# lzhangbj/DualVar

Hardware: AMD Instinct MI355X
Metric: clips/sec (whole node), S3D-G 8x112^2 SimCLR pretrain step (higher is better)
Workload: dtype fp32

## Files before the change

dualvar_amd/csrc/batchnorm.hip:

```cpp
#include "streaming.hpp"

namespace {

struct BnFinalize {
  const float* gamma; const float* beta; float eps, momentum;
  float* running_mean; float* running_var; float* mean; float* invstd; float* scale; float* shift;
};
template <typename F>
__device__ __forceinline__ void bn_finalize_channel(const F& f, int c, float mean, float M2, float cnt) {
  const float var = M2 / cnt;
  const float invstd = rsqrtf(var + f.eps);
  f.mean[c] = mean;
  f.invstd[c] = invstd;
  const float sc = f.gamma[c] * invstd;
  f.scale[c] = sc;
  f.shift[c] = f.beta[c] - mean * sc;
  if (f.running_mean) {
    f.running_mean[c] = (1.f - f.momentum) * f.running_mean[c] + f.momentum * mean;
    const float unbiased = cnt > 1.f ? M2 / (cnt - 1.f) : var;
    f.running_var[c] = (1.f - f.momentum) * f.running_var[c] + f.momentum * unbiased;
  }
}
__device__ __forceinline__ void bn_combine_ranks(const float* stats, int R, int stride, int C, int c, float& mean, float& M2, float& cnt) {
  float n = 0.f, S = 0.f;
  for (int r = 0; r < R; ++r) { n += stats[r * stride + 2 * C]; S += stats[r * stride + c]; }
  const float mu = S / n;
  float q = 0.f;
  for (int r = 0; r < R; ++r) {
    float n_r = stats[r * stride + 2 * C];
    float d = stats[r * stride + c] / n_r - mu;
    q += stats[r * stride + C + c] + n_r * d * d;
  }
// ... 101 lines not shown
      if (res) o += r[e];
      if (flags & DV_RELU) o = fmaxf(o, 0.f);
      v[e] = (c0 + e < C) ? o : 0.f;
    }
    Pack16<T>::store(y + (size_t)row * ldy + c0, v);
  }
}

template <typename T>
__global__ void bn_apply_kernel(const T* __restrict__ x, int ldx, const float* __restrict__ scale,
                                const float* __restrict__ shift, const T* __restrict__ res, int ldr,
                                T* __restrict__ y, int ldy, uint32_t total, int C, FastDiv fcv, int flags) {
  bn_apply_body<T>(x, ldx, scale, shift, res, ldr, y, ldy, total, C, fcv, flags, blockIdx.x, gridDim.x);
}

template <typename T>
__global__ void bn_apply_multi_kernel(const dv_bn_item* __restrict__ items, int n) {
  uint32_t bid = blockIdx.x, nblk;
  const int i = find_item(n, bid, nblk, [&](int k) { return items[k].blk_apply; });
  const dv_bn_item& it = items[i];
  constexpr int V = DT<T>::VEC;
  const int CP = (it.C + 7) & ~7;
  bn_apply_body<T>((const T*)it.x, it.ldx, it.scale, it.shift, (const T*)it.residual, it.ldr, (T*)it.y, it.ldy,
                   (uint32_t)(it.M * (CP / V)), it.C, make_fastdiv((uint32_t)(CP / V)), it.fwd_flags, bid, nblk);
}

struct GateOnLoad {
  const float* g; const float* dm; FastDiv fS; int ldg; float invS;
};

template <typename T>
struct PlainDy {
  static constexpr int V = DT<T>::VEC, kRows = 0;
  static constexpr bool kPooled = false;
  struct Pend {};
  const T* dy; int lddy;
  __device__ __forceinline__ void load(int64_t r, int c0, float (&g)[V], Pend&) const { Pack16<T>::load(dy + r * lddy + c0, g); }
  __device__ __forceinline__ void finish(int64_t, int, float (&)[V], Pend&) const {}
};

template <typename T, bool ROW_FIRST>
struct GatedDy {
  static constexpr int V = DT<T>::VEC, kRows = V == 4 ? 2 : 1;
  static constexpr bool kPooled = false;
  struct Pend { float gv[V], dv[V]; };
  const T* dy; int lddy; GateOnLoad ga;
  __device__ __forceinline__ void gate_row(int64_t r, int c0, Pend& p) const {
    const size_t go = (size_t)fd_div((uint32_t)r, ga.fS) * ga.ldg;
    load_params<V>(ga.g + go, c0, p.gv);
    load_params<V>(ga.dm + go, c0, p.dv);
  }
  __device__ __forceinline__ void load(int64_t r, int c0, float (&g)[V], Pend& p) const {
    if (ROW_FIRST && ga.g) gate_row(r, c0, p);
    Pack16<T>::load(dy + r * lddy + c0, g);
  }
  __device__ __forceinline__ void finish(int64_t r, int c0, float (&g)[V], Pend& p) const {
    if (!ga.g) return;
    if (!ROW_FIRST) gate_row(r, c0, p);
#pragma unroll
    for (int e = 0; e < V; ++e) g[e] = as_stored<T>(gate_grad(g[e], p.gv[e], p.dv[e], ga.invS));
  }
};

template <typename T>
__global__ __launch_bounds__(kThreads) void bn_bwd_reduce_kernel(const T* __restrict__ dy, int lddy, const T* __restrict__ y, int ldy,
                                     const T* __restrict__ x, int ldx, const float* __restrict__ mean,
                                     const float* __restrict__ invstd, int64_t M, int C, int CP, int flags,
                                     int64_t rows_per_block, float* __restrict__ sums_all, int n_rep, float* __restrict__ ws) {
  bn_bwd_reduce_body<T>(PlainDy<T>{dy, lddy}, y, ldy, x, ldx, mean, invstd, M, C, CP, flags, rows_per_block, sums_all, n_rep,
                        blockIdx.x, nullptr, nullptr, ws, gridDim.x);
}

template <typename T>
__global__ __launch_bounds__(kThreads) void bn_bwd_reduce_multi_kernel(const dv_bn_item* __restrict__ items, int n) {
  uint32_t bid = blockIdx.x, nblk;
  const int i = find_item(n, bid, nblk, [&](int k) { return items[k].blk_red; });
  const dv_bn_item& it = items[i];
  const int CP = (it.C + 7) & ~7;
  const int64_t rpb = (it.M + nblk - 1) / nblk;
  bn_bwd_reduce_body<T>(PlainDy<T>{(const T*)it.dy, it.lddy}, (const T*)it.y, it.ldy, (const T*)it.x, it.ldx, it.mean,
                        it.invstd, it.M, it.C, CP, it.bwd_flags, rpb, it.sums, it.n_rep, bid, it.scale, it.shift, it.red_ws, nblk);
}

__device__ __forceinline__ GateOnLoad gate_of_item(const int32_t* __restrict__ gate_off, int i, const float* g, const float* dm,
                                                   const FastDiv& fS, int ldg) {
  const int off = gate_off[i];
  GateOnLoad ga;
  ga.g = off >= 0 ? g + off : nullptr;
  ga.dm = off >= 0 ? dm + off : nullptr;
  ga.fS = fS; ga.ldg = ldg; ga.invS = 1.f / (float)fS.d;
  return ga;
}

template <typename T>
__global__ __launch_bounds__(kThreads) void bn_bwd_reduce_multi_gated_kernel(const dv_bn_item* __restrict__ items, int n,
                                                                            const int32_t* __restrict__ gate_off,
                                                                            const float* __restrict__ g, const float* __restrict__ dm,
                                                                            FastDiv fS, int ldg) {
  uint32_t bid = blockIdx.x, nblk;
  const int i = find_item(n, bid, nblk, [&](int k) { return items[k].blk_red; });
  const dv_bn_item& it = items[i];
  const int CP = (it.C + 7) & ~7;
  const int64_t rpb = (it.M + nblk - 1) / nblk;
  bn_bwd_reduce_body<T>(GatedDy<T, true>{(const T*)it.dy, it.lddy, gate_of_item(gate_off, i, g, dm, fS, ldg)}, (const T*)it.y, it.ldy,
                        (const T*)it.x, it.ldx, it.mean, it.invstd, it.M, it.C, CP, it.bwd_flags, rpb, it.sums, it.n_rep, bid,
                        it.scale, it.shift, it.red_ws, nblk);
}

template <typename T>
__global__ void bn_bwd_apply_kernel(const T* __restrict__ dy, int lddy, const T* __restrict__ y, int ldy,
                                    const T* __restrict__ x, int ldx, const float* __restrict__ mean,
                                    const float* __restrict__ invstd, const float* __restrict__ gamma,
                                    const float* __restrict__ sums_g, int rep_g, float inv_count, float dscale,
                                    float* dgamma, float* dbeta, T* __restrict__ dx, int lddx,
                                    T* __restrict__ dres, int lddres, uint32_t total, int C, int CP, FastDiv fcv,
                                    int flags) {
  bn_bwd_apply_body<T>(PlainDy<T>{dy, lddy}, y, ldy, x, ldx, mean, invstd, gamma, sums_g, rep_g, inv_count, dscale, dgamma,
                       dbeta, dx, lddx, dres, lddres, total, C, CP, fcv, flags, blockIdx.x, gridDim.x, nullptr, nullptr);
}

template <typename T>
__global__ void bn_bwd_apply_multi_kernel(const dv_bn_item* __restrict__ items, int n) {
  uint32_t bid = blockIdx.x, nblk;
  const int i = find_item(n, bid, nblk, [&](int k) { return items[k].blk_bapply; });
  const dv_bn_item& it = items[i];
  constexpr int V = DT<T>::VEC;
  const int CP = (it.C + 7) & ~7;
  bn_bwd_apply_body<T>(PlainDy<T>{(const T*)it.dy, it.lddy}, (const T*)it.y, it.ldy, (const T*)it.x, it.ldx, it.mean, it.invstd,
                       it.gamma, it.sums, it.n_rep, it.inv_count, it.dparam_scale, it.dgamma, it.dbeta, (T*)it.dx, it.lddx,
                       (T*)it.dres, it.lddres, (uint32_t)(it.M * (CP / V)), it.C, CP, make_fastdiv((uint32_t)(CP / V)),
                       it.bwd_flags, bid, nblk, it.scale, it.shift);
}

template <typename T>
__global__ void bn_bwd_apply_multi_gated_kernel(const dv_bn_item* __restrict__ items, int n, const int32_t* __restrict__ gate_off,
                                                const float* __restrict__ g, const float* __restrict__ dm, FastDiv fS, int ldg) {
  uint32_t bid = blockIdx.x, nblk;
  const int i = find_item(n, bid, nblk, [&](int k) { return items[k].blk_bapply; });
  const dv_bn_item& it = items[i];
  constexpr int V = DT<T>::VEC;
  const int CP = (it.C + 7) & ~7;
  bn_bwd_apply_body<T>(GatedDy<T, false>{(const T*)it.dy, it.lddy, gate_of_item(gate_off, i, g, dm, fS, ldg)}, (const T*)it.y, it.ldy,
                       (const T*)it.x, it.ldx, it.mean, it.invstd, it.gamma, it.sums, it.n_rep, it.inv_count, it.dparam_scale,
                       it.dgamma, it.dbeta, (T*)it.dx, it.lddx, (T*)it.dres, it.lddres, (uint32_t)(it.M * (CP / V)), it.C, CP,
                       make_fastdiv((uint32_t)(CP / V)), it.bwd_flags, bid, nblk, it.scale, it.shift);
}

}

__global__ void bn_eval_coeffs_kernel(const float* __restrict__ gamma, const float* __restrict__ beta,
                                      const float* __restrict__ rm, const float* __restrict__ rv, float eps, int C, int CP,
                                      float* __restrict__ scale, float* __restrict__ shift) {
  const int c = blockIdx.x * blockDim.x + threadIdx.x;
  if (c >= CP) return;
  float sc = 0.f, sh = 0.f;
  if (c < C) {
    sc = gamma[c] * rsqrtf(rv[c] + eps);
    sh = beta[c] - rm[c] * sc;
  }
  scale[c] = sc;
  shift[c] = sh;
}

extern "C" int dv_bn_eval_coeffs(const float* gamma, const float* beta, const float* running_mean, const float* running_var,
                                 float eps, int32_t C, float* scale, float* shift, void* stream) {
  if (!gamma || !beta || !running_mean || !running_var || !scale || !shift || C <= 0) return DV_EINVAL;
  const int CP = cp8(C);
  hipLaunchKernelGGL(bn_eval_coeffs_kernel, dim3((CP + 127) / 128), dim3(128), 0, ST(stream), gamma, beta, running_mean,
                     running_var, eps, C, CP, scale, shift);
  return dv_launch_status();
}

__global__ void bn_rows_partials_kernel(const float* __restrict__ x, int ldx, int M, int C, float* __restrict__ part) {
  const int c = blockIdx.x * blockDim.x + threadIdx.x;
  if (c >= C) return;
// ... 189 lines not shown
```

dualvar_amd/csrc/conv.hip:

```cpp
#include "conv_common.hpp"
#include "../../include/dualvar_conv_pair.h"

static int w3_rows(int n) { return (n + 127) / 128 * 128; }
static int64_t w3_bytes(int n, int ktot) { return (int64_t)((ktot + 15) / 16) * 2 * w3_rows(n) * 48; }

namespace {
__global__ __launch_bounds__(256) void pack_w3_kernel(const float* __restrict__ base, unsigned char* __restrict__ out_base,
                                                      const dv_w3_desc* __restrict__ descs, const int2* __restrict__ block_map) {
  const int2 bm = block_map[blockIdx.x];
  const dv_w3_desc d = descs[bm.x];
  const int npad = (d.N + 127) / 128 * 128;
  const long long unit = (long long)bm.y + threadIdx.x;
  const long long units = (long long)((d.Ktot + 15) / 16) * 2 * npad;
  if (unit >= units) return;
  const int n = (int)(unit % npad);
  const int kh = (int)(unit / npad), k0 = (kh >> 1) * 16 + (kh & 1) * 8;
  float v[8];
#pragma unroll
  for (int e = 0; e < 8; ++e) v[e] = (n < d.N && k0 + e < d.Ktot) ? base[d.src_off + (long long)n * d.Ktot + k0 + e] : 0.f;
  const Split3 s3 = split3(v);
  bf16x8* o = reinterpret_cast<bf16x8*>(out_base + d.dst_off + unit * 48);
  o[0] = s3.hi; o[1] = s3.mid; o[2] = s3.lo;
}
}

extern "C" int64_t dv_w3_bytes(int32_t rows, int32_t ktot) { return rows > 0 && ktot > 0 ? w3_bytes(rows, ktot) : 0; }

extern "C" int dv_pack_w3(const float* base, void* out_base, const dv_w3_desc* descs, const int32_t* block_map, int32_t n_blocks,
                          void* stream) {
  if (!base || !out_base || !descs || !block_map || n_blocks <= 0) return DV_EINVAL;
  hipLaunchKernelGGL(pack_w3_kernel, dim3(n_blocks), dim3(256), 0, (hipStream_t)stream, base, (unsigned char*)out_base, descs,
                     reinterpret_cast<const int2*>(block_map));
  return dv_launch_status();
}

static int pick_bn(int np) {
  if (np <= 32) return 32;
  if (np <= 64) return 64;
  int w128 = (np + 127) / 128 * 128, w64 = (np + 63) / 64 * 64;
  return (w128 <= w64) ? 128 : 64;
}

static int pick_bm(int M, int ntn) {
  return ((int64_t)((M + 127) / 128) * ntn >= 1024) ? 128 : 64;
}

static void pick_tile(int dtype, int M, int NP, int& bm, int& bn) {
  bn = pick_bn(NP);
  const int ntn = (NP + bn - 1) / bn;
  bm = pick_bm(M, ntn);
  if (dtype == DV_F32 && !f32_exact() && bm == 128 && bn == 64 && (int64_t)((M + 255) / 256) * ntn >= 512) bm = 256;
  constexpr int fill = 256;
  if (bm == 64) {
// ... 559 lines not shown
```

dualvar_amd/csrc/elementwise.hip:

```cpp
#include "streaming.hpp"

namespace {

template <typename T>
__global__ void ingest_kernel(const float* __restrict__ x, T* __restrict__ y, int N, int C, int T_, int H, int W,
                              int64_t sxn, int ldy, const float* mean3, const float* istd3,
                              const int* perm, int n_seg, int pad, int Hp, int Wp) {
  const int64_t total = (int64_t)N * T_ * H * W;
  const int64_t plane = (int64_t)H * W;
  const int seg = n_seg > 0 ? T_ / n_seg : T_;
  for (int64_t i = blockIdx.x * (int64_t)blockDim.x + threadIdx.x; i < total; i += (int64_t)gridDim.x * blockDim.x) {
    int64_t hw = i % plane;
    int64_t nt = i / plane;
    int t = (int)(nt % T_);
    int n = (int)(nt / T_);
    int ts = t;
    if (perm) ts = perm[n * n_seg + t / seg] * seg + t % seg;
    const float* src = x + (int64_t)n * sxn + (int64_t)ts * plane + hw;
    float v[4] = {0.f, 0.f, 0.f, 0.f};
    for (int c = 0; c < C && c < 4; ++c) {
      float a = src[(int64_t)c * T_ * plane];
      if (mean3) a = (a - mean3[c]) * istd3[c];
      v[c] = a;
    }
// ... 42 lines not shown
  if (row >= R) return;
  const int lane = threadIdx.x & 63;
  float s = 0.f;
  for (int d = lane; d < D; d += 64) { float v = x[(size_t)row * D + d]; s += v * v; }
  s = wave_sum(s);
  const float nrm = fmaxf(sqrtf(s), eps);
  for (int d = lane; d < D; d += 64) y[(size_t)row * D + d] = x[(size_t)row * D + d] / nrm;
  if (lane == 0) norm[row] = nrm;
}
__global__ void l2norm_bwd_kernel(const float* __restrict__ dy, const float* __restrict__ y,
                                  const float* __restrict__ norm, int R, int D, float* __restrict__ dx) {
  const int row = blockIdx.x * (blockDim.x >> 6) + (threadIdx.x >> 6);
  if (row >= R) return;
  const int lane = threadIdx.x & 63;
  float s = 0.f;
  for (int d = lane; d < D; d += 64) s += dy[(size_t)row * D + d] * y[(size_t)row * D + d];
  s = wave_sum(s);
  const float inv = 1.f / norm[row];
  for (int d = lane; d < D; d += 64)
    dx[(size_t)row * D + d] = (dy[(size_t)row * D + d] - y[(size_t)row * D + d] * s) * inv;
}
__global__ void relu_bwd_kernel(const float* __restrict__ dy, const float* __restrict__ y, int64_t n, float* __restrict__ dx) {
  for (int64_t i = blockIdx.x * (int64_t)blockDim.x + threadIdx.x; i < n; i += (int64_t)gridDim.x * blockDim.x)
    dx[i] = y[i] > 0.f ? dy[i] : 0.f;
}
__global__ void mean_kernel(const float* __restrict__ x, int n, float* __restrict__ out) {
  __shared__ float sh[8];
  float s = 0.f;
  for (int i = threadIdx.x; i < n; i += blockDim.x) s += x[i];
  s = block_sum(s, sh);
  if (threadIdx.x == 0) out[0] = s / (float)n;
}

template <typename CT>
__global__ void pack_dgrad_kernel(const float* __restrict__ master, CT* __restrict__ dst,
                                  const dv_pack_desc* __restrict__ descs, const int* __restrict__ bmap) {
  const dv_pack_desc d = descs[bmap[2 * blockIdx.x]];
  const int c = bmap[2 * blockIdx.x + 1];
  const int rowlen = d.taps * d.cout_pitch;
  const float* src = master + d.src_off;
  CT* out = dst + d.dst_off + (int64_t)c * rowlen;
  for (int i = threadIdx.x; i < rowlen; i += blockDim.x) {
    const int tap = i / d.cout_pitch, n = i % d.cout_pitch;
    float v = 0.f;
    if (n < d.Cout) v = src[((int64_t)n * d.taps + tap) * d.cin_pitch + c];
    out[i] = (CT)v;
  }
}

}

extern "C" int dv_abi_version(void) { return DV_ABI_VERSION; }

extern "C" int dv_check_device(void) {
  int dev = 0;
  if (hipGetDevice(&dev) != hipSuccess) return DV_EUNSUPPORTED;
  hipDeviceProp_t prop;
  if (hipGetDeviceProperties(&prop, dev) != hipSuccess) return DV_EUNSUPPORTED;
  const char* a = prop.gcnArchName;
  return (a[0] == 'g' && a[1] == 'f' && a[2] == 'x' && a[3] == '9' && a[4] == '5' && a[5] == '0') ? DV_OK : DV_EUNSUPPORTED;
}

extern "C" int dv_ingest_ncdhw(int32_t dtype, const float* x, void* y, int32_t N, int32_t C, int32_t T_, int32_t H,
                               int32_t W, int64_t sxn, int32_t ldy, const float* mean3, const float* istd3,
                               const int32_t* perm, int32_t n_seg, void* stream) {
  if (!x || !y || N <= 0 || C <= 0 || C > 4 || ldy < 4 || ldy % 4) return DV_EINVAL;
  if (perm && (n_seg <= 0 || T_ % n_seg)) return DV_EINVAL;
  if ((mean3 == nullptr) != (istd3 == nullptr)) return DV_EINVAL;
  const int64_t total = (int64_t)N * T_ * H * W;
  DISPATCH_T(dtype, hipLaunchKernelGGL((ingest_kernel<T>), dim3(grid_for(total)), dim3(kThreads), 0, ST(stream), x,
                                       (T*)y, N, C, T_, H, W, sxn, ldy, mean3, istd3, perm, n_seg, 0, H, W));
  return dv_launch_status();
}

extern "C" int dv_ingest_ncdhw_pad(int32_t dtype, const float* x, void* y, int32_t N, int32_t C, int32_t T_, int32_t H,
                                   int32_t W, int64_t sxn, int32_t ldy, const float* mean3, const float* istd3,
                                   const int32_t* perm, int32_t n_seg, int32_t pad, void* stream) {
  if (!x || !y || N <= 0 || C <= 0 || C > 4 || ldy < 4 || ldy % 4 || pad < 0) return DV_EINVAL;
  if (perm && (n_seg <= 0 || T_ % n_seg)) return DV_EINVAL;
// ... 69 lines not shown
```

dualvar_amd/csrc/pool.hip:

```cpp
#include "streaming.hpp"

namespace {

__device__ __forceinline__ uint32_t xcd_block() { return (blockIdx.x & 7u) * (gridDim.x >> 3) + (blockIdx.x >> 3); }
static inline int grid8_for(int64_t work_items, int max_blocks) { return (grid_for(work_items, max_blocks) + 7) & ~7; }

struct PoolArgs {
  int N, Ti, Hi, Wi, C, CP;
  int To, Ho, Wo;
  int kt, kh, kw, st, sh, sw, pt, ph, pw;
  int ldx, ldy;
  FastDiv fcv, fWo, fHo, fTo, fWi, fHi, fTi;
};

template <typename T>
__global__ void maxpool_fwd_kernel(PoolArgs a, const T* __restrict__ x, T* __restrict__ y, uint8_t* __restrict__ idx) {
  constexpr int V = DT<T>::VEC;
  const uint32_t CV = a.fcv.d;
  const uint32_t total = (uint32_t)a.N * a.To * a.Ho * a.Wo * CV;
  for (uint32_t i = xcd_block() * blockDim.x + threadIdx.x; i < total; i += gridDim.x * blockDim.x) {
    uint32_t m, cvi, q, wo_, ho_, to_, n_;
    fd_divmod(i, a.fcv, m, cvi);
    const int c0 = (int)cvi * V;
    fd_divmod(m, a.fWo, q, wo_);
// ... 187 lines not shown
                                            uint32_t m_in, int c0, float (&g)[DT<T>::VEC]) {
  constexpr int V = DT<T>::VEC;
  uint32_t q, wi_, hi_, ti_, n_;
  fd_divmod(m_in, a.fWi, q, wi_);
  fd_divmod(q, a.fHi, q, hi_);
  fd_divmod(q, a.fTi, n_, ti_);
  const int n = (int)n_;
  const int st1 = a.st - 1, sh1 = a.sh - 1, sw1 = a.sw - 1;
  const int tn = (int)ti_ + a.pt, hn = (int)hi_ + a.ph, wn = (int)wi_ + a.pw;
  const int t_hi = min(tn >> st1, a.To - 1), t_lo = max((tn - a.kt + 1 + st1) >> st1, 0);
  const int h_hi = min(hn >> sh1, a.Ho - 1), h_lo = max((hn - a.kh + 1 + sh1) >> sh1, 0);
  const int w_hi = min(wn >> sw1, a.Wo - 1), w_lo = max((wn - a.kw + 1 + sw1) >> sw1, 0);
  for (int to = t_hi; to >= t_lo; --to) {
    const int dt = tn - to * a.st;
    for (int ho = h_hi; ho >= h_lo; --ho) {
      const int dh = hn - ho * a.sh;
      for (int wo = w_hi; wo >= w_lo; --wo) {
        const uint32_t tap = (uint32_t)((dt * a.kh + dh) * a.kw + wn - wo * a.sw);
        const int64_t mo = (int64_t)((n * a.To + to) * a.Ho + ho) * a.Wo + wo;
        float d[V];
        Pack16<T>::load(dyp + mo * a.ldy + c0, d);
        const uint8_t* ip = idx + mo * a.CP + c0;
#pragma unroll
        for (int e = 0; e < V; ++e)
          if (ip[e] == tap) g[e] += d[e];
      }
    }
  }
}

template <typename T>
struct PooledDy {
  static constexpr int V = DT<T>::VEC, kRows = 0;
  static constexpr bool kPooled = true;
  struct Pend {};
  const PoolArgs& a; const T* dyp; const uint8_t* idx;
  __device__ __forceinline__ void load(int64_t r, int c0, float (&g)[V], Pend&) const {
#pragma unroll
    for (int e = 0; e < V; ++e) g[e] = 0.f;
    pool_gather<T>(a, dyp, idx, (uint32_t)r, c0, g);
  }
  __device__ __forceinline__ void finish(int64_t, int, float (&)[V], Pend&) const {}
};

template <typename T>
__global__ __launch_bounds__(kThreads) void bn_bwd_reduce_maxpool_kernel(PoolArgs a, const T* __restrict__ dyp, const uint8_t* __restrict__ idx,
                                             const T* __restrict__ x, const float* __restrict__ mean,
                                             const float* __restrict__ invstd, const float* __restrict__ scale,
                                             const float* __restrict__ shift, int64_t M, int C, int CP, int64_t rows_per_block,
                                             float* __restrict__ sums_all, int n_rep) {
  bn_bwd_reduce_body<T>(PooledDy<T>{a, dyp, idx}, nullptr, 0, x, a.ldx, mean, invstd, M, C, CP, 0, rows_per_block, sums_all,
                        n_rep, blockIdx.x, scale, shift, nullptr, gridDim.x);
}

template <typename T>
__global__ void bn_bwd_apply_maxpool_kernel(PoolArgs a, const T* __restrict__ dyp, const uint8_t* __restrict__ idx,
                                            const T* __restrict__ x, const float* __restrict__ mean,
                                            const float* __restrict__ invstd, const float* __restrict__ gamma,
                                            const float* __restrict__ scale, const float* __restrict__ shift,
                                            const float* __restrict__ sums_g, int rep_g, float inv_count, float dscale,
                                            float* dgamma, float* dbeta, T* __restrict__ dx, int lddx, uint32_t total, int C,
                                            int CP) {
  bn_bwd_apply_body<T>(PooledDy<T>{a, dyp, idx}, nullptr, 0, x, a.ldx, mean, invstd, gamma, sums_g, rep_g, inv_count, dscale,
                       dgamma, dbeta, dx, lddx, nullptr, 0, total, C, CP, a.fcv, 0, blockIdx.x, gridDim.x, scale, shift);
}

struct PoolTileArgs {
  int N, T, H, W, C, CP, ldx, ldy;
  int nth, ntw, ncc, cpv;
  uint32_t groups, per_xcd;
  FastDiv fcc, ftw, fth;
  int accumulate;
};

__device__ __forceinline__ uint32_t key_f32(uint32_t x) { return x ^ ((uint32_t)((int32_t)x >> 31) | 0x80000000u); }
// ... 473 lines not shown
```

dualvar_amd/csrc/streaming.hpp:

```cpp
#pragma once
#include "common.hpp"
#include "ordered_fold.hpp"

namespace {

constexpr int kThreads = 256;

__device__ __forceinline__ float block_sum(float v, float* sh ) {
  v = wave_sum(v);
  const int w = threadIdx.x >> 6;
  __syncthreads();
  if ((threadIdx.x & 63) == 0) sh[w] = v;
  __syncthreads();
  float r = 0.f;
  for (int i = 0; i < (int)(blockDim.x >> 6); ++i) r += sh[i];
  return r;
}

template <int V>
__device__ __forceinline__ void load_params(const float* __restrict__ p, int c0, float (&v)[V]) {
#pragma unroll
  for (int q = 0; q < V / 4; ++q) {
    f32x4 t = *reinterpret_cast<const f32x4*>(p + c0 + 4 * q);
    v[4 * q] = t.x; v[4 * q + 1] = t.y; v[4 * q + 2] = t.z; v[4 * q + 3] = t.w;
  }
}

__device__ __forceinline__ float bn_affine(float x, float sc, float sh) { return x * sc + sh; }
template <typename T>
__device__ __forceinline__ float as_stored(float v) { return DT<T>::to_f(DT<T>::from_f(v)); }
template <typename T>
__device__ __forceinline__ float bn_relu_stored(float x, float sc, float sh) { return as_stored<T>(fmaxf(bn_affine(x, sc, sh), 0.f)); }
__device__ __forceinline__ float gate_grad(float dy, float g, float dm, float invS) { return dy * g + dm * invS; }

struct NoPre { __device__ __forceinline__ void operator()(int) const {} };

template <int V, int NS, int UNROLL = 0, typename F, typename W, typename Pre = NoPre>
__device__ __forceinline__ void column_reduce(int64_t r_begin, int64_t r_end, int CP, F f, W write, Pre pre = Pre()) {
  __shared__ float lds[kThreads * V * NS > 4096 ? 4096 : kThreads * V * NS];
  const int CV = CP / V;
  for (int cvb = 0; cvb < CV; cvb += kThreads) {
    const int cvc = min(kThreads, CV - cvb);
    int rg = kThreads / cvc;
    while (rg > 1 && rg * cvc * V * NS > 4096) rg >>= 1;
    const int t = threadIdx.x;
    const int my_cv = t % cvc, my_rg = t / cvc;
    float acc[NS][V];
#pragma unroll
    for (int s = 0; s < NS; ++s)
#pragma unroll
      for (int e = 0; e < V; ++e) acc[s][e] = 0.f;
    if (my_rg < rg) {
      pre((cvb + my_cv) * V);
#pragma unroll(UNROLL ? UNROLL : V == 4 ? 4 : 2)
      for (int64_t r = r_begin + my_rg; r < r_end; r += rg) f(r, (cvb + my_cv) * V, acc);
    }
    __syncthreads();
    if (rg == 1 && cvc * V * NS > 4096) {
      if (my_rg < rg) write((cvb + my_cv) * V, acc);
    } else {
      if (my_rg < rg) {
#pragma unroll
        for (int s = 0; s < NS; ++s)
#pragma unroll
          for (int e = 0; e < V; ++e) lds[((my_rg * NS + s) * cvc + my_cv) * V + e] = acc[s][e];
      }
      __syncthreads();
      for (int n = rg; n > 1;) {
        const int half = (n + 1) >> 1;
        if (my_rg < rg && my_rg + half < n) {
#pragma unroll
          for (int s = 0; s < NS; ++s)
#pragma unroll
            for (int e = 0; e < V; ++e)
              lds[((my_rg * NS + s) * cvc + my_cv) * V + e] += lds[(((my_rg + half) * NS + s) * cvc + my_cv) * V + e];
        }
        __syncthreads();
        n = half;
      }
      if (t < cvc) {
#pragma unroll
        for (int s = 0; s < NS; ++s)
#pragma unroll
          for (int e = 0; e < V; ++e) acc[s][e] = lds[(s * cvc + t) * V + e];
        write((cvb + t) * V, acc);
      }
    }
    __syncthreads();
// ... 1 lines not shown
}

static inline int64_t ordered_fold_floats(int nblk, int CP) { return fold_rows_total(nblk) * 2 * CP + fold_ticket_words(nblk); }

__device__ __forceinline__ void fold_rows(const float* __restrict__ rows, int n, int NO, int C, int CP, float* __restrict__ dst,
                                          bool coherent_dst) {
  for (int i = threadIdx.x; i < NO; i += blockDim.x) {
    const int c = i < CP ? i : i - CP;
    const float t = c < C ? fold_in_order<32>(rows + i, n, NO) : 0.f;
    if (coherent_dst) coherent_store(dst + i, t);
    else dst[i] = t;
  }
}
__device__ __forceinline__ void ordered_fold(float* __restrict__ ws, uint32_t bid, uint32_t nblk, int C, int CP, float* __restrict__ out) {
  __shared__ uint32_t last;
  const int NO = 2 * CP;
  constexpr uint32_t gfold = kFoldGroup;
  const uint32_t ngrp = fold_groups((int)nblk), grp = bid / gfold;
  const uint32_t gsize = min(gfold, nblk - grp * gfold);
  float* grows = ws + (size_t)nblk * NO;
  uint32_t* tick = reinterpret_cast<uint32_t*>(grows + (size_t)ngrp * NO);
  if (!took_last_ticket(tick + grp, gsize, &last)) return;
  if (ngrp == 1) {
    fold_rows(ws, (int)gsize, NO, C, CP, out, false);
    clear_ticket(tick);
    return;
  }
  fold_rows(ws + (size_t)grp * gfold * NO, (int)gsize, NO, C, CP, grows + (size_t)grp * NO, true);
  clear_ticket(tick + grp);
  if (!took_last_ticket(tick + ngrp, ngrp, &last)) return;
  fold_rows(grows, (int)ngrp, NO, C, CP, out, false);
  clear_ticket(tick + ngrp);
}

template <typename T, typename Src>
__device__ __forceinline__ void bn_bwd_reduce_body(const Src& src, const T* __restrict__ y, int ldy,
                                                   const T* __restrict__ x, int ldx, const float* __restrict__ mean,
                                                   const float* __restrict__ invstd, int64_t M, int C, int CP, int flags,
                                                   int64_t rows_per_block, float* __restrict__ sums_all, int n_rep,
                                                   uint32_t bid, const float* __restrict__ scale,
                                                   const float* __restrict__ shift, float* __restrict__ ws, uint32_t nblk) {
  constexpr int V = DT<T>::VEC;
  if (Src::kPooled) { flags = DV_MASK_FROM_X; ws = nullptr; }
  float* sums = ws ? ws + (size_t)bid * 2 * CP : sums_all + (size_t)(bid % n_rep) * 2 * CP;
  const int64_t r0 = (int64_t)bid * rows_per_block;
  const int64_t r1 = min(M, r0 + rows_per_block);
  const bool mask = !(flags & DV_NO_RELU_MASK);
  const bool fromx = mask && (flags & DV_MASK_FROM_X);
  float mu[V], is[V], sc[V], sh[V];
  column_reduce<V, 2, Src::kRows>(
      r0, r1, CP,
      [&](int64_t r, int c0, float(&acc)[2][V]) {
        float g[V], yy[V], xx[V];
        typename Src::Pend pend;
        src.load(r, c0, g, pend);
        if (mask && !fromx) Pack16<T>::load(y + r * ldy + c0, yy);
        Pack16<T>::load(x + r * ldx + c0, xx);
        src.finish(r, c0, g, pend);
#pragma unroll
        for (int e = 0; e < V; ++e) {
          const float act = fromx ? bn_affine(xx[e], sc[e], sh[e]) : yy[e];
          float gg = (mask && !(act > 0.f)) ? 0.f : g[e];
          acc[0][e] += gg;
          acc[1][e] += gg * (xx[e] - mu[e]) * is[e];
        }
      },
      [&](int c0, float(&acc)[2][V]) {
#pragma unroll
        for (int e = 0; e < V; ++e)
          if (c0 + e < C) {
            if (ws) { coherent_store(sums + c0 + e, acc[0][e]); coherent_store(sums + CP + c0 + e, acc[1][e]); }
            else { atomicAdd(sums + c0 + e, acc[0][e]); atomicAdd(sums + CP + c0 + e, acc[1][e]); }
          }
      },
      [&](int c0) {
        load_params<V>(mean, c0, mu);
        load_params<V>(invstd, c0, is);
        if (fromx) { load_params<V>(scale, c0, sc); load_params<V>(shift, c0, sh); }
      });
  if (ws) ordered_fold(ws, bid, nblk, C, CP, sums_all);
}

template <typename T, typename Src>
__device__ __forceinline__ void bn_bwd_apply_body(const Src& src, const T* __restrict__ y, int ldy,
                                                  const T* __restrict__ x, int ldx, const float* __restrict__ mean,
                                                  const float* __restrict__ invstd, const float* __restrict__ gamma,
                                                  const float* __restrict__ sums_g, int rep_g, float inv_count,
                                                  float dscale, float* dgamma, float* dbeta, T* __restrict__ dx,
                                                  int lddx, T* __restrict__ dres, int lddres, uint32_t total, int C,
                                                  int CP, const FastDiv& fcv, int flags, uint32_t bid, uint32_t nblk,
                                                  const float* __restrict__ scale, const float* __restrict__ shift) {
  constexpr int V = DT<T>::VEC;
  if (Src::kPooled) { flags = DV_MASK_FROM_X; dres = nullptr; }
  extern __shared__ __attribute__((aligned(16))) float coef[];
  const bool fromx = !(flags & DV_NO_RELU_MASK) && (flags & DV_MASK_FROM_X);
  if (bid == 0 && dgamma) {
    for (int c = threadIdx.x; c < C; c += blockDim.x) {
      float sb = 0.f, sg = 0.f;
      for (int r = 0; r < rep_g; ++r) { sb += sums_g[(size_t)r * 2 * CP + c]; sg += sums_g[(size_t)r * 2 * CP + CP + c]; }
      dbeta[c] += dscale * sb;
      dgamma[c] += dscale * sg;
    }
  }
  for (int c = threadIdx.x; c < CP; c += blockDim.x) {
    float k1 = 0.f, k2 = 0.f, k3 = 0.f;
    if (c < C) {
      float sg = 0.f, sgx = 0.f;
      for (int r = 0; r < rep_g; ++r) { sg += sums_g[(size_t)r * 2 * CP + c]; sgx += sums_g[(size_t)r * 2 * CP + CP + c]; }
      k1 = gamma[c] * invstd[c];
      k2 = -k1 * invstd[c] * sgx * inv_count;
      k3 = -k1 * sg * inv_count - k2 * mean[c];
    }
    coef[c] = k1; coef[CP + c] = k2; coef[2 * CP + c] = k3;
    if (fromx) { coef[3 * CP + c] = c < C ? scale[c] : 0.f; coef[4 * CP + c] = c < C ? shift[c] : 0.f; }
  }
  __syncthreads();
  const uint32_t CV = fcv.d;
  const bool mask = !(flags & DV_NO_RELU_MASK);
  for (uint32_t i = bid * blockDim.x + threadIdx.x; i < total; i += nblk * blockDim.x) {
    const uint32_t row = fd_div(i, fcv);
    const int c0 = (int)(i - row * CV) * V;
    float g[V], yy[V], xx[V], o[V], ro[V], k1[V], k2[V], k3[V], sc[V], sh[V];
    typename Src::Pend pend;
    src.load(row, c0, g, pend);
    if (mask && !fromx) Pack16<T>::load(y + (size_t)row * ldy + c0, yy);
    Pack16<T>::load(x + (size_t)row * ldx + c0, xx);
    if (dres && (flags & DV_ACCUM)) Pack16<T>::load(dres + (size_t)row * lddres + c0, ro);
    src.finish(row, c0, g, pend);
    load_params<V>(coef, c0, k1);
    load_params<V>(coef + CP, c0, k2);
    load_params<V>(coef + 2 * CP, c0, k3);
    if (fromx) { load_params<V>(coef + 3 * CP, c0, sc); load_params<V>(coef + 4 * CP, c0, sh); }
#pragma unroll
    for (int e = 0; e < V; ++e) {
      const float act = fromx ? bn_affine(xx[e], sc[e], sh[e]) : yy[e];
      const float gg = (mask && !(act > 0.f)) ? 0.f : g[e];
      o[e] = k1[e] * gg + k2[e] * xx[e] + k3[e];
      if (dres) ro[e] = c0 + e >= C ? 0.f : (flags & DV_ACCUM) ? ro[e] + gg : gg;
    }
    Pack16<T>::store(dx + (size_t)row * lddx + c0, o);
    if (dres) Pack16<T>::store(dres + (size_t)row * lddres + c0, ro);
  }
}

}

#define DISPATCH_T(dtype, ...)                                  \
  do {                                                          \
    if ((dtype) == DV_F32) { typedef float T; __VA_ARGS__; }    \
    else if ((dtype) == DV_BF16) { typedef bf16_t T; __VA_ARGS__; } \
    else return DV_EUNSUPPORTED;                                \
  } while (0)

static inline int cp8(int c) { return (c + 7) & ~7; }
```

dualvar_amd/engine.py:

```python
import ctypes as C
import os

import torch
import torch.distributed as dist

from . import _lib as L
from . import rccl
from . import ops
from ._lib import DV_MASK_FROM_X
from .ops import DV_ACCUM, DV_BF16, DV_BIAS, DV_F32, DV_NO_RELU_MASK, DV_RELU, DV_SIGMOID, DV_STATS, Act, cp8


BN_REPLICAS = 1


def _align8(n):
    return (n + 7) & ~7


WGRAD_SIDE_STREAM = os.environ.get('DUALVAR_WGRAD_STREAM', '1') != '0'
SIDE_LAUNCHES = ('conv_wgrad', 'gate_db')
WGRAD_BATCH = int(os.environ.get('DUALVAR_WGRAD_BATCH', '4'))
WGRAD_FLUSH_FLOPS = float(os.environ.get('DUALVAR_WGRAD_FLUSH_GFLOP', '3')) * 1e9
WGRAD_EARLY_RATIO = 0.5
# ... 226 lines not shown
            if v != self._versions:
                self._dirty = True
        if not self._dirty:
            if self._fp8_stale:
                self._refresh_fp8()
            return
        if self.dtype == DV_BF16 and not self._cast_done:
            ops.call('dv_cast_arena', DV_BF16, self.master, self.cc, self.total)
        if self._n_pack_blocks:
            ops.call('dv_pack_dgrad_weights', self.dtype, self.master, self.wd, self._pack_descs, self._pack_map,
                     self._n_pack_blocks)
        self._refresh_w3()
        self._refresh_fp8()
        self._dirty = False
        self._cast_done = False
        self._versions = self._version_sum()

    def _w3_setup(self, device, dtype):
        self.w3 = self.wd3 = None
        self._w3_jobs = []
        for s_ in self.slots + self.merged:
            s_.w3_off = s_.wd3_off = -1
        if dtype != DV_F32 or L.f32_exact():
            return
        lib = L.load()
        convs = [s_ for s_ in self.slots + self.merged if s_.kind in ('conv', 'merged')]

        def table(rows_k, src_of, attr):
            arr, bmap, off = (L.W3Desc * len(rows_k))(), [], 0
            for i, (s_, rows, ktot) in enumerate(rows_k):
                setattr(s_, attr, off)
                arr[i].src_off, arr[i].dst_off, arr[i].N, arr[i].Ktot = src_of(s_), off, rows, ktot
                nbytes = int(lib.dv_w3_bytes(rows, ktot))
                bmap += [(i, u) for u in range(0, nbytes // 48, 256)]
                off += nbytes
            return (torch.zeros(max(off, 16), dtype=torch.uint8, device=device),
                    torch.frombuffer(bytearray(bytes(arr)), dtype=torch.uint8).to(device),
                    torch.tensor(bmap, dtype=torch.int32).to(device), len(bmap))
        fwd = [(s_, s_.Cout, s_.taps * s_.cin_pitch) for s_ in convs]
        self.w3, d1, m1, n1 = table(fwd, lambda s_: s_.off, 'w3_off')
        self._w3_jobs.append(('master', self.w3, d1, m1, n1))
        bwd = [(s_, s_.Cin, s_.taps * s_.cout_pitch) for s_ in convs if s_.wd_off >= 0]
        if bwd:
            self.wd3, d2, m2, n2 = table(bwd, lambda s_: s_.wd_off, 'wd3_off')
            self._w3_jobs.append(('wd', self.wd3, d2, m2, n2))

    def _refresh_w3(self):
        for src, out, descs, bmap, n in getattr(self, '_w3_jobs', ()):
            base = self.master if src == 'master' else self.wd
            ops.call('dv_pack_w3', base, out, descs, bmap, n)

    def fp8_weights(self, s):
        e = self._fp8.get(id(s))
        if e is None:
            dev = self.master.device
            e = (s, torch.zeros(s.Cout, s.cin_pitch, dtype=torch.uint8, device=dev), torch.ones(1, device=dev),
                 torch.zeros(s.Cin, s.cout_pitch, dtype=torch.uint8, device=dev), torch.ones(1, device=dev))
            self._fp8[id(s)] = e
            self._fp8_stale = True
        return e[1:]

    def _refresh_fp8(self):
        if not self._fp8:
            return
        lib = L.load()
        if self._fp8_ws is None:
            self._fp8_ws = torch.empty(lib.dv_quantize_fp8_workspace() // 4, dtype=torch.float32, device=self.master.device)
# ... 1231 lines not shown
```

dualvar_amd/ops.py:

```python
import ctypes as C

import torch

from . import _lib as L
from ._lib import DV_ACCUM, DV_BF16, DV_BIAS, DV_F32, DV_NO_RELU_MASK, DV_RELU, DV_SIGMOID, DV_STATS

TORCH_DTYPE = {DV_F32: torch.float32, DV_BF16: torch.bfloat16}
ESIZE = {DV_F32: 4, DV_BF16: 2}


def cp8(c):
    return (c + 7) & ~7


def stream_ptr():
    return torch.cuda.current_stream().cuda_stream


class Act:
    __slots__ = ('buf', 'N', 'T', 'H', 'W', 'C', 'ld', 'off', 'dtype', 'grad', 'cpitch', 'producer', 'hw_pad')

    def __init__(self, buf, N, T, H, W, C, ld, off, dtype, cpitch=None):
        self.buf, self.N, self.T, self.H, self.W, self.C, self.ld, self.off, self.dtype = buf, N, T, H, W, C, ld, off, dtype
        self.cpitch = cpitch if cpitch is not None else cp8(C)
# ... 98 lines not shown
    L.check(lib.dv_conv3d_fwd_bn_in(C.byref(d), _p(x_bn), C.byref(bn), _p(w), _p(y), _p(stats), stream_ptr()), 'dv_conv3d_fwd_bn_in')


def conv_wgrad_bn_in(d, x_bn, bn, dy, dw, workspace=None):
    lib = L.load()
    need = wgrad_workspace_bytes(d)
    if workspace is None and need:
        workspace = torch.empty(need, dtype=torch.uint8, device=dw.device)
    nbytes = workspace.numel() * workspace.element_size() if workspace is not None else 0
    L.check(lib.dv_conv3d_wgrad_bn_in(C.byref(d), _p(x_bn), C.byref(bn), _p(dy), _p(dw), _p(workspace), nbytes, stream_ptr()),
            'dv_conv3d_wgrad_bn_in')


def quantize_fp8(x, M, C, ld, fmt, dtype, q=None, scale=None, workspace=None):
    lib = L.load()
    dev = x.device if isinstance(x, torch.Tensor) else x.buf.device
    q = torch.empty(M, C, dtype=torch.uint8, device=dev) if q is None else q
    scale = torch.empty(1, dtype=torch.float32, device=dev) if scale is None else scale
    if workspace is None:
        workspace = torch.empty(lib.dv_quantize_fp8_workspace() // 4, dtype=torch.float32, device=dev)
    L.check(lib.dv_quantize_fp8(dtype, _p(x), M, C, ld, fmt, _p(q), q.stride(0), _p(scale), _p(workspace), stream_ptr()),
            'dv_quantize_fp8')
    return q, scale


def conv_fwd_fp8(d, x8, w8, sx, sw, y, stats):
    L.check(L.load().dv_conv3d_fwd_fp8(C.byref(d), _p(x8), _p(w8), _p(sx), _p(sw), _p(y), _p(stats), stream_ptr()), 'dv_conv3d_fwd_fp8')


def conv_dgrad_fp8(d, dy8, wd8, sdy, sw, dx):
    L.check(L.load().dv_conv3d_dgrad_fp8(C.byref(d), _p(dy8), _p(wd8), _p(sdy), _p(sw), _p(dx), stream_ptr()), 'dv_conv3d_dgrad_fp8')


def pack_w3(w):
    lib = L.load()
    rows, ktot = w.shape
    nbytes = int(lib.dv_w3_bytes(rows, ktot))
    out = torch.zeros(nbytes, dtype=torch.uint8, device=w.device)
    d = (L.W3Desc * 1)()
    d[0].src_off, d[0].dst_off, d[0].N, d[0].Ktot = 0, 0, rows, ktot
    descs = torch.frombuffer(bytearray(bytes(d)), dtype=torch.uint8).to(w.device)
    bmap = torch.tensor([(0, u) for u in range(0, nbytes // 48, 256)], dtype=torch.int32, device=w.device)
    call('dv_pack_w3', w.contiguous(), out, descs, bmap, bmap.shape[0])
    return out


def stat_tiles(d):
    return L.load().dv_conv3d_stat_tiles(C.byref(d))


def tile_rows(d):
    return L.load().dv_conv3d_tile_rows(C.byref(d))


def pool_desc(dtype, x, y, k, s, p):
    d = L.PoolDesc()
    d.dtype = dtype
    d.N, d.Ti, d.Hi, d.Wi, d.C = x.N, x.T, x.H, x.W, x.C
    d.To, d.Ho, d.Wo = y.T, y.H, y.W
    d.kt, d.kh, d.kw = k
    d.st, d.sh, d.sw = s
    d.pt, d.ph, d.pw = p
    d.ldx, d.ldy = x.ld, y.ld
    return d


def call(name, *args):
    lib = L.load()
    conv = []
    for a in args:
        if isinstance(a, (Act, torch.Tensor)) or a is None:
            conv.append(_p(a))
        elif isinstance(a, C.Structure):
            conv.append(C.byref(a))
        else:
# ... 29 lines not shown
```

Before: 8156.

## Coalesce weight packing via LDS transposes and segment gate loads in BN backward

```diff
diff --git a/dualvar_amd/csrc/batchnorm.hip b/dualvar_amd/csrc/batchnorm.hip
--- a/dualvar_amd/csrc/batchnorm.hip
+++ b/dualvar_amd/csrc/batchnorm.hip
@@ -1,3 +1,4 @@
+#include <type_traits>
 #include "streaming.hpp"
 
 namespace {
@@ -165,33 +166,47 @@
 template <typename T>
 struct PlainDy {
   static constexpr int V = DT<T>::VEC, kRows = 0;
-  static constexpr bool kPooled = false;
+  static constexpr bool kPooled = false, kSegmented = false;
   struct Pend {};
+  struct Seg {};
   const T* dy; int lddy;
   __device__ __forceinline__ void load(int64_t r, int c0, float (&g)[V], Pend&) const { Pack16<T>::load(dy + r * lddy + c0, g); }
-  __device__ __forceinline__ void finish(int64_t, int, float (&)[V], Pend&) const {}
+  __device__ __forceinline__ void finish(int64_t, int, float (&)[V], Pend&, const Seg&) const {}
 };
 
-template <typename T, bool ROW_FIRST>
+enum { kGateSegments, kGateRowFirst, kGateRowLast };
+template <typename T, int MODE>
 struct GatedDy {
-  static constexpr int V = DT<T>::VEC, kRows = V == 4 ? 2 : 1;
-  static constexpr bool kPooled = false;
-  struct Pend { float gv[V], dv[V]; };
+  static constexpr int V = DT<T>::VEC, kRows = MODE == kGateSegments ? 3 : V == 4 ? 2 : 1;
+  static constexpr bool kPooled = false, kSegmented = MODE == kGateSegments;
+  struct Vecs { float gv[V], dv[V]; };
+  struct None {};
+  using Pend = typename std::conditional<kSegmented, None, Vecs>::type;
+  using Seg = typename std::conditional<kSegmented, Vecs, None>::type;
   const T* dy; int lddy; GateOnLoad ga;
-  __device__ __forceinline__ void gate_row(int64_t r, int c0, Pend& p) const {
-    const size_t go = (size_t)fd_div((uint32_t)r, ga.fS) * ga.ldg;
+  __device__ __forceinline__ void gate_row(uint32_t n, int c0, Vecs& p) const {
+    const size_t go = (size_t)n * ga.ldg;
     load_params<V>(ga.g + go, c0, p.gv);
     load_params<V>(ga.dm + go, c0, p.dv);
   }
+  __device__ __forceinline__ int64_t enter(int64_t sb, int64_t r_end, int c0, Vecs& s) const {
+    if (!ga.g) return r_end;
+    const uint32_t n = fd_div((uint32_t)sb, ga.fS);
+    gate_row(n, c0, s);
+    return min(r_end, (int64_t)(n + 1) * ga.fS.d);
+  }
   __device__ __forceinline__ void load(int64_t r, int c0, float (&g)[V], Pend& p) const {
-    if (ROW_FIRST && ga.g) gate_row(r, c0, p);
+    if constexpr (MODE == kGateRowFirst) { if (ga.g) gate_row(fd_div((uint32_t)r, ga.fS), c0, p); }
     Pack16<T>::load(dy + r * lddy + c0, g);
   }
-  __device__ __forceinline__ void finish(int64_t r, int c0, float (&g)[V], Pend& p) const {
+  __device__ __forceinline__ void finish(int64_t r, int c0, float (&g)[V], Pend& p, const Seg& s) const {
     if (!ga.g) return;
-    if (!ROW_FIRST) gate_row(r, c0, p);
+    if constexpr (MODE == kGateRowLast) gate_row(fd_div((uint32_t)r, ga.fS), c0, p);
 #pragma unroll
-    for (int e = 0; e < V; ++e) g[e] = as_stored<T>(gate_grad(g[e], p.gv[e], p.dv[e], ga.invS));
+    for (int e = 0; e < V; ++e) {
+      if constexpr (kSegmented) g[e] = as_stored<T>(gate_grad(g[e], s.gv[e], s.dv[e], ga.invS));
+      else g[e] = as_stored<T>(gate_grad(g[e], p.gv[e], p.dv[e], ga.invS));
+    }
   }
 };
 
@@ -235,7 +250,7 @@
   const dv_bn_item& it = items[i];
   const int CP = (it.C + 7) & ~7;
   const int64_t rpb = (it.M + nblk - 1) / nblk;
-  bn_bwd_reduce_body<T>(GatedDy<T, true>{(const T*)it.dy, it.lddy, gate_of_item(gate_off, i, g, dm, fS, ldg)}, (const T*)it.y, it.ldy,
+  bn_bwd_reduce_body<T>(GatedDy<T, sizeof(T) == 4 ? kGateSegments : kGateRowFirst>{(const T*)it.dy, it.lddy, gate_of_item(gate_off, i, g, dm, fS, ldg)}, (const T*)it.y, it.ldy,
                         (const T*)it.x, it.ldx, it.mean, it.invstd, it.M, it.C, CP, it.bwd_flags, rpb, it.sums, it.n_rep, bid,
                         it.scale, it.shift, it.red_ws, nblk);
 }
@@ -273,7 +288,7 @@
   const dv_bn_item& it = items[i];
   constexpr int V = DT<T>::VEC;
   const int CP = (it.C + 7) & ~7;
-  bn_bwd_apply_body<T>(GatedDy<T, false>{(const T*)it.dy, it.lddy, gate_of_item(gate_off, i, g, dm, fS, ldg)}, (const T*)it.y, it.ldy,
+  bn_bwd_apply_body<T>(GatedDy<T, kGateRowLast>{(const T*)it.dy, it.lddy, gate_of_item(gate_off, i, g, dm, fS, ldg)}, (const T*)it.y, it.ldy,
                        (const T*)it.x, it.ldx, it.mean, it.invstd, it.gamma, it.sums, it.n_rep, it.inv_count, it.dparam_scale,
                        it.dgamma, it.dbeta, (T*)it.dx, it.lddx, (T*)it.dres, it.lddres, (uint32_t)(it.M * (CP / V)), it.C, CP,
                        make_fastdiv((uint32_t)(CP / V)), it.bwd_flags, bid, nblk, it.scale, it.shift);
diff --git a/dualvar_amd/csrc/conv.hip b/dualvar_amd/csrc/conv.hip
--- a/dualvar_amd/csrc/conv.hip
+++ b/dualvar_amd/csrc/conv.hip
@@ -5,20 +5,43 @@
 static int64_t w3_bytes(int n, int ktot) { return (int64_t)((ktot + 15) / 16) * 2 * w3_rows(n) * 48; }
 
 namespace {
+constexpr int kW3Rows = 64, kW3Pitch = 36;
 __global__ __launch_bounds__(256) void pack_w3_kernel(const float* __restrict__ base, unsigned char* __restrict__ out_base,
                                                       const dv_w3_desc* __restrict__ descs, const int2* __restrict__ block_map) {
+  __shared__ __attribute__((aligned(16))) float t[kW3Rows * kW3Pitch];
   const int2 bm = block_map[blockIdx.x];
   const dv_w3_desc d = descs[bm.x];
-  const int npad = (d.N + 127) / 128 * 128;
-  const long long unit = (long long)bm.y + threadIdx.x;
-  const long long units = (long long)((d.Ktot + 15) / 16) * 2 * npad;
-  if (unit >= units) return;
-  const int n = (int)(unit % npad);
-  const int kh = (int)(unit / npad), k0 = (kh >> 1) * 16 + (kh & 1) * 8;
-  float v[8];
+  const int npad = (d.N + 127) / 128 * 128, nrb = npad / kW3Rows, nkh = (d.Ktot + 15) / 16 * 2;
+  const int ks = bm.y / nrb, n0 = (bm.y - ks * nrb) * kW3Rows;
+  if (bm.y < 0 || ks * 4 >= nkh) return;
+  const float* src = base + d.src_off;
+  const bool vec = reinterpret_cast<uintptr_t>(src) % 16 == 0 && d.Ktot % 4 == 0;
+  const int lr = threadIdx.x >> 3, lk = (threadIdx.x & 7) * 4;
 #pragma unroll
-  for (int e = 0; e < 8; ++e) v[e] = (n < d.N && k0 + e < d.Ktot) ? base[d.src_off + (long long)n * d.Ktot + k0 + e] : 0.f;
+  for (int p = 0; p < kW3Rows / 32; ++p) {
+    const int row = lr + p * 32, n = n0 + row, k = ks * 32 + lk;
+    float4 v = make_float4(0.f, 0.f, 0.f, 0.f);
+    if (n < d.N) {
+      const float* s = src + (long long)n * d.Ktot + k;
+      if (vec) {
+        if (k < d.Ktot) v = *reinterpret_cast<const float4*>(s);
+      } else {
+        if (k + 0 < d.Ktot) v.x = s[0];
+        if (k + 1 < d.Ktot) v.y = s[1];
+        if (k + 2 < d.Ktot) v.z = s[2];
+        if (k + 3 < d.Ktot) v.w = s[3];
+      }
+    }
+    *reinterpret_cast<float4*>(t + row * kW3Pitch + lk) = v;
+  }
+  __syncthreads();
+  const int q = threadIdx.x >> 6, r = threadIdx.x & 63, kh = ks * 4 + q;
+  if (kh >= nkh) return;
+  const float4 a = *reinterpret_cast<const float4*>(t + r * kW3Pitch + q * 8);
+  const float4 b = *reinterpret_cast<const float4*>(t + r * kW3Pitch + q * 8 + 4);
+  const float v[8] = {a.x, a.y, a.z, a.w, b.x, b.y, b.z, b.w};
   const Split3 s3 = split3(v);
+  const long long unit = (long long)kh * npad + n0 + r;
   bf16x8* o = reinterpret_cast<bf16x8*>(out_base + d.dst_off + unit * 48);
   o[0] = s3.hi; o[1] = s3.mid; o[2] = s3.lo;
 }
diff --git a/dualvar_amd/csrc/elementwise.hip b/dualvar_amd/csrc/elementwise.hip
--- a/dualvar_amd/csrc/elementwise.hip
+++ b/dualvar_amd/csrc/elementwise.hip
@@ -98,19 +98,57 @@
   if (threadIdx.x == 0) out[0] = s / (float)n;
 }
 
+constexpr int kPackC = 32, kPackN = 64, kPackPitch = kPackN + 1;
 template <typename CT>
-__global__ void pack_dgrad_kernel(const float* __restrict__ master, CT* __restrict__ dst,
-                                  const dv_pack_desc* __restrict__ descs, const int* __restrict__ bmap) {
+__global__ __launch_bounds__(kThreads) void pack_dgrad_kernel(const float* __restrict__ master, CT* __restrict__ dst,
+                                                              const dv_pack_desc* __restrict__ descs, const int* __restrict__ bmap) {
+  constexpr int V = 16 / sizeof(CT);
+  constexpr int LPC = kPackN / V, CPP = kThreads / LPC;
+  __shared__ float t[kPackC * kPackPitch];
   const dv_pack_desc d = descs[bmap[2 * blockIdx.x]];
   const int c = bmap[2 * blockIdx.x + 1];
-  const int rowlen = d.taps * d.cout_pitch;
+  if (c < 0 || c >= d.Cin) return;
   const float* src = master + d.src_off;
-  CT* out = dst + d.dst_off + (int64_t)c * rowlen;
-  for (int i = threadIdx.x; i < rowlen; i += blockDim.x) {
-    const int tap = i / d.cout_pitch, n = i % d.cout_pitch;
-    float v = 0.f;
-    if (n < d.Cout) v = src[((int64_t)n * d.taps + tap) * d.cin_pitch + c];
-    out[i] = (CT)v;
+  if (reinterpret_cast<uintptr_t>(src) % 16 || d.cin_pitch % 4 || reinterpret_cast<uintptr_t>(dst + d.dst_off) % 16 || d.cout_pitch % V) {
+    const int rowlen = d.taps * d.cout_pitch;
+    CT* out = dst + d.dst_off + (int64_t)c * rowlen;
+    for (int i = threadIdx.x; i < rowlen; i += blockDim.x) {
+      const int tap = i / d.cout_pitch, n = i % d.cout_pitch;
+      float v = 0.f;
+      if (n < d.Cout) v = src[((int64_t)n * d.taps + tap) * d.cin_pitch + c];
+      out[i] = (CT)v;
+    }
+    return;
+  }
+  const int c0 = c & ~(kPackC - 1), gsz = min(kPackC, d.Cin - c0);
+  const int ntile = (d.cout_pitch + kPackN - 1) / kPackN, tiles = d.taps * ntile;
+  const int lr = threadIdx.x >> 3, lc = (threadIdx.x & 7) * 4;
+  const int sc = threadIdx.x / LPC, sn = (threadIdx.x % LPC) * V;
+  for (int tile = c - c0; tile < tiles; tile += gsz) {
+    const int tap = tile / ntile, n0 = (tile - tap * ntile) * kPackN;
+#pragma unroll
+    for (int p = 0; p < kPackN / 32; ++p) {
+      const int row = lr + p * 32, n = n0 + row;
+      float4 v = make_float4(0.f, 0.f, 0.f, 0.f);
+      if (n < d.Cout && c0 + lc < d.cin_pitch)
+        v = *reinterpret_cast<const float4*>(src + ((int64_t)n * d.taps + tap) * d.cin_pitch + c0 + lc);
+      t[(lc + 0) * kPackPitch + row] = v.x;
+      t[(lc + 1) * kPackPitch + row] = v.y;
+      t[(lc + 2) * kPackPitch + row] = v.z;
+      t[(lc + 3) * kPackPitch + row] = v.w;
+    }
+    __syncthreads();
+#pragma unroll
+    for (int cl = sc; cl < kPackC; cl += CPP) {
+      if (c0 + cl < d.Cin && n0 + sn < d.cout_pitch) {
+        alignas(16) CT o[V];
+#pragma unroll
+        for (int e = 0; e < V; ++e) o[e] = (CT)t[cl * kPackPitch + sn + e];
+        CT* out = dst + d.dst_off + ((int64_t)(c0 + cl) * d.taps + tap) * d.cout_pitch + n0 + sn;
+        *reinterpret_cast<uint4*>(out) = *reinterpret_cast<const uint4*>(o);
+      }
+    }
+    __syncthreads();
   }
 }
 
diff --git a/dualvar_amd/csrc/pool.hip b/dualvar_amd/csrc/pool.hip
--- a/dualvar_amd/csrc/pool.hip
+++ b/dualvar_amd/csrc/pool.hip
@@ -243,15 +243,16 @@
 template <typename T>
 struct PooledDy {
   static constexpr int V = DT<T>::VEC, kRows = 0;
-  static constexpr bool kPooled = true;
+  static constexpr bool kPooled = true, kSegmented = false;
   struct Pend {};
+  struct Seg {};
   const PoolArgs& a; const T* dyp; const uint8_t* idx;
   __device__ __forceinline__ void load(int64_t r, int c0, float (&g)[V], Pend&) const {
 #pragma unroll
     for (int e = 0; e < V; ++e) g[e] = 0.f;
     pool_gather<T>(a, dyp, idx, (uint32_t)r, c0, g);
   }
-  __device__ __forceinline__ void finish(int64_t, int, float (&)[V], Pend&) const {}
+  __device__ __forceinline__ void finish(int64_t, int, float (&)[V], Pend&, const Seg&) const {}
 };
 
 template <typename T>
diff --git a/dualvar_amd/csrc/streaming.hpp b/dualvar_amd/csrc/streaming.hpp
--- a/dualvar_amd/csrc/streaming.hpp
+++ b/dualvar_amd/csrc/streaming.hpp
@@ -34,9 +34,10 @@
 __device__ __forceinline__ float gate_grad(float dy, float g, float dm, float invS) { return dy * g + dm * invS; }
 
 struct NoPre { __device__ __forceinline__ void operator()(int) const {} };
-
-template <int V, int NS, int UNROLL = 0, typename F, typename W, typename Pre = NoPre>
-__device__ __forceinline__ void column_reduce(int64_t r_begin, int64_t r_end, int CP, F f, W write, Pre pre = Pre()) {
+struct NoSeg { static constexpr bool kOn = false; };
+
+template <int V, int NS, int UNROLL = 0, typename F, typename W, typename Pre = NoPre, typename Seg = NoSeg>
+__device__ __forceinline__ void column_reduce(int64_t r_begin, int64_t r_end, int CP, F f, W write, Pre pre = Pre(), Seg seg = Seg()) {
   __shared__ float lds[kThreads * V * NS > 4096 ? 4096 : kThreads * V * NS];
   const int CV = CP / V;
   for (int cvb = 0; cvb < CV; cvb += kThreads) {
@@ -52,8 +53,17 @@
       for (int e = 0; e < V; ++e) acc[s][e] = 0.f;
     if (my_rg < rg) {
       pre((cvb + my_cv) * V);
+      if constexpr (Seg::kOn) {
+        int64_t r = r_begin + my_rg;
+        for (int64_t sb = r_begin; sb < r_end;) {
+          sb = seg(sb, r_end, (cvb + my_cv) * V);
+#pragma unroll(UNROLL ? UNROLL : V == 4 ? 4 : 2)
+          for (; r < sb; r += rg) f(r, (cvb + my_cv) * V, acc);
+        }
+      } else {
 #pragma unroll(UNROLL ? UNROLL : V == 4 ? 4 : 2)
       for (int64_t r = r_begin + my_rg; r < r_end; r += rg) f(r, (cvb + my_cv) * V, acc);
+      }
     }
     __syncthreads();
     if (rg == 1 && cvc * V * NS > 4096) {
@@ -121,6 +131,13 @@
   fold_rows(grows, (int)ngrp, NO, C, CP, out, false);
   clear_ticket(tick + ngrp);
 }
+
+template <typename Src>
+struct SrcSegments {
+  static constexpr bool kOn = Src::kSegmented;
+  const Src& src; typename Src::Seg& seg;
+  __device__ __forceinline__ int64_t operator()(int64_t sb, int64_t r_end, int c0) const { return src.enter(sb, r_end, c0, seg); }
+};
 
 template <typename T, typename Src>
 __device__ __forceinline__ void bn_bwd_reduce_body(const Src& src, const T* __restrict__ y, int ldy,
@@ -137,6 +154,7 @@
   const bool mask = !(flags & DV_NO_RELU_MASK);
   const bool fromx = mask && (flags & DV_MASK_FROM_X);
   float mu[V], is[V], sc[V], sh[V];
+  typename Src::Seg seg;
   column_reduce<V, 2, Src::kRows>(
       r0, r1, CP,
       [&](int64_t r, int c0, float(&acc)[2][V]) {
@@ -145,7 +163,7 @@
         src.load(r, c0, g, pend);
         if (mask && !fromx) Pack16<T>::load(y + r * ldy + c0, yy);
         Pack16<T>::load(x + r * ldx + c0, xx);
-        src.finish(r, c0, g, pend);
+        src.finish(r, c0, g, pend, seg);
 #pragma unroll
         for (int e = 0; e < V; ++e) {
           const float act = fromx ? bn_affine(xx[e], sc[e], sh[e]) : yy[e];
@@ -166,7 +184,8 @@
         load_params<V>(mean, c0, mu);
         load_params<V>(invstd, c0, is);
         if (fromx) { load_params<V>(scale, c0, sc); load_params<V>(shift, c0, sh); }
-      });
+      },
+      SrcSegments<Src>{src, seg});
   if (ws) ordered_fold(ws, bid, nblk, C, CP, sums_all);
 }
 
@@ -211,11 +230,12 @@
     const int c0 = (int)(i - row * CV) * V;
     float g[V], yy[V], xx[V], o[V], ro[V], k1[V], k2[V], k3[V], sc[V], sh[V];
     typename Src::Pend pend;
+    typename Src::Seg seg;
     src.load(row, c0, g, pend);
     if (mask && !fromx) Pack16<T>::load(y + (size_t)row * ldy + c0, yy);
     Pack16<T>::load(x + (size_t)row * ldx + c0, xx);
     if (dres && (flags & DV_ACCUM)) Pack16<T>::load(dres + (size_t)row * lddres + c0, ro);
-    src.finish(row, c0, g, pend);
+    src.finish(row, c0, g, pend, seg);
     load_params<V>(coef, c0, k1);
     load_params<V>(coef + CP, c0, k2);
     load_params<V>(coef + 2 * CP, c0, k3);
diff --git a/dualvar_amd/engine.py b/dualvar_amd/engine.py
--- a/dualvar_amd/engine.py
+++ b/dualvar_amd/engine.py
@@ -282,7 +282,7 @@
                 setattr(s_, attr, off)
                 arr[i].src_off, arr[i].dst_off, arr[i].N, arr[i].Ktot = src_of(s_), off, rows, ktot
                 nbytes = int(lib.dv_w3_bytes(rows, ktot))
-                bmap += [(i, u) for u in range(0, nbytes // 48, 256)]
+                bmap += ops.w3_block_map(i, rows, ktot)
                 off += nbytes
             return (torch.zeros(max(off, 16), dtype=torch.uint8, device=device),
                     torch.frombuffer(bytearray(bytes(arr)), dtype=torch.uint8).to(device),
diff --git a/dualvar_amd/ops.py b/dualvar_amd/ops.py
--- a/dualvar_amd/ops.py
+++ b/dualvar_amd/ops.py
@@ -154,6 +154,11 @@
     L.check(L.load().dv_conv3d_dgrad_fp8(C.byref(d), _p(dy8), _p(wd8), _p(sdy), _p(sw), _p(dx), stream_ptr()), 'dv_conv3d_dgrad_fp8')
 
 
+def w3_block_map(i, rows, ktot):
+    row_blocks, k_spans = (rows + 127) // 128 * 2, (ktot + 31) // 32
+    return [(i, b) for b in range(k_spans * row_blocks)]
+
+
 def pack_w3(w):
     lib = L.load()
     rows, ktot = w.shape
@@ -162,7 +167,7 @@
     d = (L.W3Desc * 1)()
     d[0].src_off, d[0].dst_off, d[0].N, d[0].Ktot = 0, 0, rows, ktot
     descs = torch.frombuffer(bytearray(bytes(d)), dtype=torch.uint8).to(w.device)
-    bmap = torch.tensor([(0, u) for u in range(0, nbytes // 48, 256)], dtype=torch.int32, device=w.device)
+    bmap = torch.tensor(w3_block_map(0, rows, ktot), dtype=torch.int32, device=w.device)
     call('dv_pack_w3', w.contiguous(), out, descs, bmap, bmap.shape[0])
     return out
 
```

Result: no change. 8202 (median of 6 runs) (+0.6%).
